# jzhoubu/vsearch

Hardware: AMD Instinct MI355X
Metric: queries/sec over 21M-doc sparse index, k=100; recall@100 vs reference (higher is better)
Workload: dtype f32

## Files before the change

### vsearch_amd/csrc/bp_quad.h

```cpp
#pragma once
#include "bp_walk.h"
#include "bp_quad_loop.h"
#include "bp_quad_asm.h"

#ifndef VS_QUAD_EPI
#define VS_QUAD_EPI 2
#endif

namespace vs {

constexpr int kQuadRows = 2048;
constexpr int kQuadQT = 8;
constexpr int kQuadPer = kBpEntCap / kScanThreads;
constexpr size_t kQuadAccBytes = (size_t)(kQuadRows / 16) * kQuadGroupDw * 4;
static_assert(kBpEntCap % kScanThreads == 0, "a thread owns a fixed number of entries");
static_assert(kQuadAccBytes >= kBpSortBytes, "the accumulator area holds the 8192-slot entry sort");
__host__ __device__ constexpr size_t quad_fixed_lds() { return kQuadAccBytes + (size_t)kBpCap * 8 + (size_t)kQuadQT * 16 + 64 * 4; }
__host__ __device__ constexpr size_t quad_cut_lds() { return quad_fixed_lds() + (size_t)(kBpEntCap + 64 + 64 * kQuadOverRead) * 8; }
__host__ __device__ constexpr size_t quad_lds_bytes() { return quad_cut_lds() + (size_t)kCutHistWords * 4; }
static_assert(quad_lds_bytes() <= (size_t)160 * 1024, "the quad walk's LDS");
static_assert(kBpCap == 2 * kScanThreads, "wg_cut_topk: two keys of the candidate buffer a thread");
static_assert(kQuadQT == 8 && (kQuadAccBytes + (size_t)kBpCap * 8) % 16 == 0, "the epilogue reads thresholds and counters 16 bytes at a time");
constexpr int kQuadListCap = 64 - 4 * kQuadOverRead, kQuadListBytes = (kQuadListCap + 4 * kQuadOverRead) * 8;
static_assert(kQuadListCap >= 16, "room for links in a wave's list");
static_assert(2 * kQuadListBytes * kScanWaves <= kBpCap * 8, "the link lists fit the sort buffer");
constexpr int kQuadLinked = kQuadCells - 2;
constexpr double kQuadMaxRatio = 3.0;
constexpr int kQuadPfLines = 384;
constexpr int kQuadPaceDefault = 0;
template <int CELLS, int LINKED>
__host__ __device__ constexpr uint32_t chunk_overflow(uint32_t n) { return n > (uint32_t)CELLS ? (n - (uint32_t)CELLS + (uint32_t)LINKED - 1u) / (uint32_t)LINKED : 0u; }
__host__ __device__ constexpr uint32_t quad_overflow_chunks(uint32_t n) { return chunk_overflow<kQuadCells, kQuadLinked>(n); }

template <int CELLS, int LINKED>
__global__ __launch_bounds__(kScanThreads) void quad_count_kernel(const uint32_t* pk_ptr, const uint4* cols, int64_t n_rows, int32_t n_cols, int32_t rows,
                                                                  uint32_t* dir, uint32_t* block_recs, unsigned long long* df_rec, unsigned long long* df_nnz,
                                                                  int32_t* overflow) {
    extern __shared__ __attribute__((aligned(16))) char smem[];
    uint32_t* cnt = reinterpret_cast<uint32_t*>(smem);
    __shared__ int scratch[32];
    const int tid = threadIdx.x;
    const int64_t n_blocks = (n_rows + rows - 1) / rows;
    const int seg = (n_cols + kScanThreads - 1) / kScanThreads;
    for (int64_t b = blockIdx.x; b < n_blocks; b += gridDim.x) {
        const int64_t r0 = b * rows, r1 = min(n_rows, r0 + rows);
        const uint32_t P0 = pk_ptr[r0], P1 = pk_ptr[r1];
        __syncthreads();
        for (int i = tid; i <= n_cols; i += kScanThreads) cnt[i] = 0;
        __syncthreads();
        for (uint32_t p = P0 + tid; p < P1; p += kScanThreads) {
            const uint4 cw = cols[p];
            const uint32_t cwv[4] = {cw.x, cw.y, cw.z, cw.w};
#pragma unroll
            for (int i = 0; i < 4; ++i) {
                atomicAdd(&cnt[cwv[i] & 0xFFFFu], 1u);
                atomicAdd(&cnt[cwv[i] >> 16], 1u);
            }
        }
        __syncthreads();
        const int i0 = min(n_cols, tid * seg), i1 = min(n_cols, i0 + seg);
        int mine = 0;
        for (int i = i0; i < i1; ++i) mine += (int)chunk_overflow<CELLS, LINKED>(cnt[i]);
        int tot = 0;
        int off = block_excl_scan(mine, scratch, tid, &tot);
        uint32_t* d = dir + (size_t)b * (n_cols + 1);
        for (int i = i0; i < i1; ++i) {
            const uint32_t c = cnt[i], r = chunk_overflow<CELLS, LINKED>(c);
            d[i] = bp_dir_pack((uint32_t)off, r);
            if (r > kBpDirRecMask || (uint32_t)off > kBpDirUnitMax) overflow[0] = 1;
            off += (int)r;
            atomicAdd(&df_rec[i], (unsigned long long)(1u + r));
            if (c) atomicAdd(&df_nnz[i], (unsigned long long)c);
        }
        if (tid == 0) { d[n_cols] = bp_dir_pack((uint32_t)tot, 0u); block_recs[b] = (uint32_t)n_cols + (uint32_t)tot; }
    }
}

template <int VS>
__global__ __launch_bounds__(kScanThreads) void quad_fill_kernel(const uint32_t* pk_ptr, const uint4* cols, const void* vals, int64_t n_rows, int32_t n_cols,
                                                                 int32_t rows, const uint32_t* dir, const unsigned long long* base, uint32_t* rec) {
    extern __shared__ __attribute__((aligned(16))) char smem[];
    uint32_t* cur = reinterpret_cast<uint32_t*>(smem);
    const int tid = threadIdx.x, lane = tid & 63, w = tid >> 6;
    const int64_t n_blocks = (n_rows + rows - 1) / rows;
    for (int64_t b = blockIdx.x; b < n_blocks; b += gridDim.x) {
        const int64_t r0 = b * rows, r1 = min(n_rows, r0 + rows);
        const uint32_t* d = dir + (size_t)b * (n_cols + 1);
        __syncthreads();
        for (int i = tid; i <= n_cols; i += kScanThreads) cur[i] = 0u;
        __syncthreads();
        uint32_t* brec = rec + (size_t)base[b] * kQuadCells;
        for (int64_t r = r0 + w; r < r1; r += kScanWaves) {
            const uint32_t p0 = pk_ptr[r], p1 = pk_ptr[r + 1];
            const uint32_t ai = quad_acc_index((uint32_t)(r - r0));
            for (uint32_t p = p0 + lane; p < p1; p += 64) {
                const uint4 cw = cols[p];
                const uint32_t cwv[4] = {cw.x, cw.y, cw.z, cw.w};
                uint32_t hb[8];
                if constexpr (VS == VM_F32) {
                    const float4* vp = reinterpret_cast<const float4*>(vals);
                    const float4 v0 = vp[2 * (size_t)p], v1 = vp[2 * (size_t)p + 1];
                    const float v[8] = {v0.x, v0.y, v0.z, v0.w, v1.x, v1.y, v1.z, v1.w};
#pragma unroll
                    for (int i = 0; i < 8; ++i) hb[i] = (uint32_t)__half_as_ushort(__float2half_rn(v[i]));
                } else {
                    const uint4 hv = reinterpret_cast<const uint4*>(vals)[p];
                    const uint32_t h4[4] = {hv.x, hv.y, hv.z, hv.w};
#pragma unroll
                    for (int i = 0; i < 8; ++i) hb[i] = (i & 1) ? (h4[i >> 1] >> 16) : (h4[i >> 1] & 0xFFFFu);
                }
#pragma unroll
                for (int i = 0; i < 8; ++i) {
                    const uint32_t c = (i & 1) ? (cwv[i >> 1] >> 16) : (cwv[i >> 1] & 0xFFFFu);
                    if (c < (uint32_t)n_cols) {
                        const uint32_t pos = atomicAdd(&cur[c], 1u);
                        const uint32_t w = d[c], m = w & kBpDirRecMask;
                        const uint32_t k = m ? min(pos / (uint32_t)kQuadLinked, m) : 0u;
                        const size_t chunk = k == 0 ? (size_t)c : (size_t)n_cols + (w >> 12) + (k - 1);
                        const uint32_t hv = (hb[i] & 0x7FFFu) ? hb[i] : 0u;
                        brec[chunk * kQuadCells + (pos - k * (uint32_t)kQuadLinked)] = ai | (hv << 16);
                    }
                }
            }
        }
        __syncthreads();
        for (int c = tid; c < n_cols; c += kScanThreads) {
            const uint32_t w = d[c], m = w & kBpDirRecMask;
            for (uint32_t k = 0; k < m; ++k) {
                const size_t chunk = k == 0 ? (size_t)c : (size_t)n_cols + (w >> 12) + (k - 1);
                const uint32_t link = (uint32_t)n_cols + (w >> 12) + k;
                brec[chunk * kQuadCells + 62] = (link >> 14) & 0x3FFFu;
                brec[chunk * kQuadCells + 63] = 0x80000000u | (link & 0x3FFFu);
            }
        }
    }
}

template <int UNUSED>
__global__ __launch_bounds__(256) void quad_arrange_kernel(uint32_t* rec, unsigned long long n_chunks) {
    extern __shared__ __attribute__((aligned(16))) char smem[];
    constexpr int LD = kQuadCells + 1;
    uint32_t* in = reinterpret_cast<uint32_t*>(smem);
    uint32_t* out = in + 256 * LD;
    const int tid = threadIdx.x;
    for (unsigned long long c0 = (unsigned long long)blockIdx.x * 256; c0 < n_chunks; c0 += (unsigned long long)gridDim.x * 256) {
        const int nc = (int)min((unsigned long long)256, n_chunks - c0);
        const uint4* src = reinterpret_cast<const uint4*>(rec + c0 * kQuadCells);
        __syncthreads();
        for (int i = tid; i < nc * 16; i += 256) {
            const uint4 v = src[i];
            uint32_t* q = in + (i >> 4) * LD + (i & 15) * 4;
            q[0] = v.x; q[1] = v.y; q[2] = v.z; q[3] = v.w;
        }
        __syncthreads();
        if (tid < nc) {
            const uint32_t* mi = in + tid * LD;
            uint32_t* mo = out + tid * LD;
            uint32_t mask[4] = {0u, 0u, 0u, 0u}, fill[4] = {0u, 0u, 0u, 0u}, room[4] = {16u, 16u, 16u, 16u};
            const bool linked = (mi[63] >> 31) != 0u;
            if (linked) {
                mo[62] = mi[62]; mo[63] = mi[63];
                mask[2] |= 1u << (mi[62] & 31u); mask[3] |= 1u << (mi[63] & 31u);
                room[2] = 15u; room[3] = 15u;
            }
            for (int i = 0; i < (linked ? kQuadLinked : kQuadCells); ++i) {
                const uint32_t p = mi[i];
                if ((p & 0x7FFF0000u) == 0u) continue;
                const uint32_t bit = 1u << (p & 31u);
                int pick = -1, any = -1;
                uint32_t best = 17u, best_any = 17u;
#pragma unroll
                for (int j = 0; j < 4; ++j) {
                    if (fill[j] < room[j] && fill[j] < best_any) { best_any = fill[j]; any = j; }
                    if (fill[j] < room[j] && !(mask[j] & bit) && fill[j] < best) { best = fill[j]; pick = j; }
                }
                if (pick < 0) pick = any;
#pragma unroll
                for (int j = 0; j < 4; ++j)
                    if (j == pick) { mo[fill[j] * 4 + j] = p; mask[j] |= bit; ++fill[j]; }
            }
#pragma unroll
            for (int j = 0; j < 4; ++j)
                while (fill[j] < room[j]) {
                    const uint32_t freeb = ~mask[j];
                    const uint32_t bk = freeb ? (uint32_t)(__ffs((int)freeb) - 1) : 0u;
                    mo[fill[j] * 4 + j] = quad_acc_index(bk);
                    mask[j] |= 1u << bk;
                    ++fill[j];
                }
        }
        __syncthreads();
        uint4* dst = reinterpret_cast<uint4*>(rec + c0 * kQuadCells);
        for (int i = tid; i < nc * 16; i += 256) {
            const uint32_t* q = out + (i >> 4) * LD + (i & 15) * 4;
            dst[i] = make_uint4(q[0], q[1], q[2], q[3]);
        }
    }
}

typedef unsigned short quad_us2 __attribute__((ext_vector_type(2)));

static_assert(kQuadRows <= 2 * kScanThreads && kQuadQT * 2 <= 32, "a thread's filter bits: two document rounds x the slots in one word");
constexpr int kQuadFiltWords = kQuadRows / 32 + 1;
constexpr size_t kQuadFiltStageBytes = (size_t)kQuadFiltWords * kQuadQT * 4;
static_assert(kQuadFiltWords * kQuadQT <= kScanThreads && quad_lds_bytes() + kQuadFiltStageBytes <= (size_t)160 * 1024, "the per-query filter stage");
template <int TM, int FL = 0>
__global__ __launch_bounds__(kScanThreads) void bp_quad_topk(KArg<BpArgs, FL> a) {
    constexpr int QT = kQuadQT;
    extern __shared__ __attribute__((aligned(16))) char smem[];
    int32_t* acc = reinterpret_cast<int32_t*>(smem);
    uint64_t* sortbuf = reinterpret_cast<uint64_t*>(smem + kQuadAccBytes);
    unsigned long long* tau = reinterpret_cast<unsigned long long*>(sortbuf + kBpCap);
    unsigned long long* upper_sh = tau + QT;
    int* scratch = reinterpret_cast<int*>(upper_sh + QT);
    unsigned int* ccnt = reinterpret_cast<unsigned int*>(scratch + 48);
    unsigned int* chi = ccnt + QT;
    uint2* desc = reinterpret_cast<uint2*>(scratch + 64);
    const uint32_t desc_lds = (uint32_t)quad_fixed_lds();
    uint32_t* cut_hist = reinterpret_cast<uint32_t*>(smem + quad_cut_lds());

    const int tid = threadIdx.x, lane = tid & 63, wv = tid >> 6;
    const int K = a.k;
    uint64_t* my_gcand = a.gcand + (size_t)blockIdx.x * QT * kBpCap;
    const int64_t n_blocks = (a.n_rows + a.rows - 1) / a.rows;
    const int64_t items = (int64_t)(a.n_tiles_dev ? a.n_tiles_dev[0] : a.n_tiles) * a.nchunk;
    const unsigned long long k_rt0 = TM ? __builtin_amdgcn_s_memrealtime() : 0ull;
    auto lds_barrier = [&]() { asm volatile("s_waitcnt lgkmcnt(0)\n\ts_barrier" ::: "memory"); };
    const uint32_t list_a = (uint32_t)kQuadAccBytes + (uint32_t)wv * 2u * kQuadListBytes, list_b = list_a + kQuadListBytes;
    const uint32_t g8 = (uint32_t)(lane >> 4) * 8u, s16 = (uint32_t)(lane & 15) * 16u;

    uint32_t pf_r = 0u, pf_R = 0u;
    if (a.pf_xcds > 0 && items <= (int64_t)gridDim.x && (int64_t)blockIdx.x < items) {
        const uint32_t X = (uint32_t)a.pf_xcds, R = ((uint32_t)items - blockIdx.x % X + X - 1u) / X;
        if (R >= 2u) { pf_r = blockIdx.x / X; pf_R = R; }
    }
    [[maybe_unused]] uint32_t n_coop = 0u;
    for (int64_t item = blockIdx.x; item < items; item += gridDim.x) {
        const int tile = (int)(item / a.nchunk), c = (int)(item % a.nchunk);
        const int q0 = a.tiles[tile].x, nq = a.tiles[tile].y;
        [[maybe_unused]] long long tm = TM ? (long long)__builtin_readcyclecounter() : 0;
        [[maybe_unused]] uint32_t tacc[6] = {0u, 0u, 0u, 0u, 0u, 0u};
        auto lap = [&](int phase) {
            if constexpr (TM != 0) {
                const long long now = (long long)__builtin_readcyclecounter();
                tacc[phase] += (uint32_t)(now - tm);
                tm = now;
            }
        };
        const int64_t b0 = (int64_t)c * a.blocks_per_chunk, b1 = min(n_blocks, b0 + a.blocks_per_chunk);
        __syncthreads();
        const int64_t e0 = a.qptr[q0], e1 = a.qptr[q0 + nq];
        const int n_ent = (int)(e1 - e0);
        const int n_static = (n_ent + 63) & ~63;
        {
            uint64_t* skey = reinterpret_cast<uint64_t*>(acc);
            for (int i = tid; i < 8192; i += kScanThreads) {
                uint64_t key = 0;
                if (i < n_ent) {
                    const int64_t e = e0 + i;
                    int qs = 0;
                    while (e >= a.qptr[q0 + qs + 1]) ++qs;
                    const float w = a.qvals[e] * a.qscale[q0 + qs];
                    key = ((uint64_t)1 << 63) | ((uint64_t)(uint32_t)a.qcols[e] << 40) | ((uint64_t)qs << 32) | (uint64_t)__float_as_uint(w);
                }
                skey[i] = key;
            }
            wg_sort_desc<kScanThreads>(skey, 8192, tid);
            for (int i = tid; i < n_static + 64 * kQuadOverRead; i += kScanThreads) {
                uint2 dsc = make_uint2(0u, 0u);
                if (i < n_ent) {
                    const uint64_t key = skey[i];
                    const uint32_t col = (uint32_t)(key >> 40) & 0xFFFFu, qs = (uint32_t)(key >> 32) & 0xFFu;
                    dsc = make_uint2((col << 8) | (qs * 16u), (uint32_t)key);
                }
                desc[i] = dsc;
            }
            __syncthreads();
        }
        for (int i = tid; i < (int)(kQuadAccBytes / 4); i += kScanThreads) acc[i] = 0;
        if (tid < QT) { tau[tid] = 0ull; ccnt[tid] = 0u; chi[tid] = 0u; }
        if (tid < QT) upper_sh[tid] = (a.upper && tid < nq) ? a.upper[q0 + tid] : ~0ull;
        __syncthreads();
        const uint32_t trips = (uint32_t)(n_static / 64);
        bool pace_off = false;
        unsigned long long base_cur = b0 < b1 ? a.base[b0] : 0ull;
        for (int64_t b = b0; b < b1 || b == b0; ++b) {
            const bool have = b < b1;
            const int rows_b = have ? (int)min((int64_t)a.rows, a.n_rows - b * a.rows) : 0;
            [[maybe_unused]] uint32_t fw0 = 0u, fw1 = 0u;
            if constexpr (FL != 0) {
                if (a.filt.ld == 0) {
                    const uint64_t bit = (uint64_t)(a.filt.bit0 + b * a.rows + tid);
                    if (tid < rows_b) fw0 = a.filt.words[bit >> 5];
                    if (tid + kScanThreads < rows_b) fw1 = a.filt.words[(bit + kScanThreads) >> 5];
                } else if (have) {
                    const int64_t w0 = (a.filt.bit0 + b * a.rows) >> 5, w1 = (a.filt.bit0 + b * a.rows + rows_b - 1) >> 5;
                    const int q = tid & (QT - 1), w = tid / QT;
                    if (w < kQuadFiltWords && q < nq && w0 + w <= w1) fw0 = a.filt.words[(size_t)(q0 + q) * (size_t)a.filt.ld + (size_t)(w0 + w)];
                }
            }
            if (have && trips > 0) {
                const char* brec = a.rec + (size_t)base_cur * kQuadChunkBytes;
                auto chain = [&](uint32_t n, uint32_t cur, uint32_t nxt) {
                    for (int depth = 0; n > 0 && depth < kQuadRows / kQuadLinked + 2; ++depth) {
                        const uint32_t n_pad = (n + 3u) & ~3u;
                        if ((uint32_t)lane < n_pad - n + 4u * kQuadOverRead)
                            reinterpret_cast<uint2*>(smem + cur)[n + (uint32_t)lane] = make_uint2(0u, 0u);
                        asm volatile("s_waitcnt lgkmcnt(0)" ::: "memory");
                        n = quad_list_asm(cur + g8, n_pad / 4u, brec, s16, nxt, (uint32_t)kQuadListCap);
                        const uint32_t t = cur; cur = nxt; nxt = t;
                    }
                };
                const uint32_t n_link = quad_walk_asm(desc_lds + (uint32_t)wv * 32u + g8, trips, brec, s16, list_a, (uint32_t)kQuadListCap);
                if (n_link <= (uint32_t)kQuadListCap) {
                    chain(n_link, list_a, list_b);
                } else {
                    constexpr uint32_t kSeg = kQuadListCap / 4;
                    for (uint32_t t0 = 0; t0 < trips; t0 += kSeg) {
                        const uint32_t n = quad_collect_asm(desc_lds + (uint32_t)wv * 32u + g8 + t0 * 512u, min(kSeg, trips - t0), brec, s16, list_a, (uint32_t)kQuadListCap);
                        chain(n, list_a, list_b);
                    }
                }
            }
            lap(1);
            if (a.pace && items <= (int64_t)gridDim.x && tid == 0 && have && !pace_off) {
                uint32_t* pc = a.pace + (size_t)c * a.blocks_per_chunk;
                const int64_t rel = b - b0;
                if (!((a.knob & 64) && blockIdx.x == 0))
                    __hip_atomic_fetch_add(pc + rel, 1u, __ATOMIC_RELAXED, __HIP_MEMORY_SCOPE_AGENT);
                if (rel >= a.pace_window) {
                    const uint32_t need = (uint32_t)(items / a.nchunk);
                    if (!pace_wait(pc + rel - a.pace_window, need)) pace_off = true;
                }
            }
            if (b + 1 < b1) base_cur = a.base[b + 1];
            if (a.gtau && tid < nq) { const unsigned long long g = a.gtau[q0 + tid]; if (g > tau[tid]) tau[tid] = g; }
            [[maybe_unused]] uint32_t fbits = 0u;
            [[maybe_unused]] uint32_t* fstage = reinterpret_cast<uint32_t*>(smem + quad_lds_bytes());
            if constexpr (FL != 0) {
                if (a.filt.ld == 0) {
#pragma unroll
                    for (int r = 0; r < 2; ++r) {
                        const uint64_t bit = (uint64_t)(a.filt.bit0 + b * a.rows + r * kScanThreads + tid);
                        if (r * kScanThreads + tid < rows_b && (((r ? fw1 : fw0) >> (bit & 31u)) & 1u)) fbits |= 0xFFu << (r * QT);
                    }
                } else if (tid < kQuadFiltWords * QT) {
                    fstage[tid] = fw0;
                }
                __builtin_amdgcn_s_waitcnt(0x0F70);
            }
            lds_barrier();
            if constexpr (FL != 0) {
                if (a.filt.ld != 0) {
                    const int64_t w0 = (a.filt.bit0 + b * a.rows) >> 5;
#pragma unroll
                    for (int r = 0; r < 2; ++r) {
                        const int d = r * kScanThreads + tid;
                        if (d < rows_b) {
                            const uint64_t bit = (uint64_t)(a.filt.bit0 + b * a.rows + d);
                            const uint4* p = reinterpret_cast<const uint4*>(fstage + ((int64_t)(bit >> 5) - w0) * QT);
                            const uint4 lo = p[0], hi = p[1];
                            const uint32_t w[QT] = {lo.x, lo.y, lo.z, lo.w, hi.x, hi.y, hi.z, hi.w};
#pragma unroll
                            for (int q = 0; q < QT; ++q) fbits |= ((w[q] >> (bit & 31u)) & 1u) << (r * QT + q);
                        }
                    }
                }
            }
            uint32_t pf = 0;
            if ((a.knob & 512) == 0 && b + 1 < b1 && trips > 0) {
                if (pf_R != 0u) {
                    const uint32_t L = pf_r + pf_R * (uint32_t)tid;
                    if (tid < a.pf_lines && L < 2u * (uint32_t)a.n_cols) {
                        const char* pl = a.rec + (size_t)base_cur * kQuadChunkBytes + (size_t)L * 128u;
                        asm volatile("global_load_dword %0, %1, off" : "=v"(pf) : "v"(pl) : "memory");
                    }
                    if constexpr (TM != 0) n_coop += 1u;
                } else if ((uint32_t)(lane >> 3) < trips) {
                    const uint32_t dx = *reinterpret_cast<const uint32_t*>(smem + desc_lds + (uint32_t)(lane >> 3) * 512u + (uint32_t)wv * 32u + (uint32_t)((lane >> 1) & 3) * 8u);
                    const char* pl = a.rec + (size_t)base_cur * kQuadChunkBytes + (dx & 0xFFFFFF00u) + (uint32_t)(lane & 1) * 128u;
                    asm volatile("global_load_dword %0, %1, off" : "=v"(pf) : "v"(pl) : "memory");
                }
            }
            lap(2);
            int32_t thr[QT];
            bool thr_stale = true;
            for (int d0 = 0; d0 < rows_b || d0 == 0; d0 += kScanThreads) {
                const int d = d0 + tid;
                const bool more = d0 + kScanThreads < rows_b;
                const uint32_t inc = more ? 1u : 0x10000u;
                if (d0 == 0 || thr_stale) {
                    const uint4* t4 = reinterpret_cast<const uint4*>(tau);
#pragma unroll
                    for (int i = 0; i < QT / 2; ++i) {
                        const uint4 t = t4[i];
                        thr[2 * i] = 2 * i < nq ? (int32_t)(t.y ^ 0x80000000u) : 0x7FFFFFFF;
                        thr[2 * i + 1] = 2 * i + 1 < nq ? (int32_t)(t.w ^ 0x80000000u) : 0x7FFFFFFF;
                    }
                    thr_stale = false;
                }
                if (d < rows_b) {
                    const int64_t row = b * a.rows + d;
                    int32_t sums[QT];
#if VS_QUAD_EPI == 0
                    int32_t* pa = acc + quad_acc_index((uint32_t)d);
#pragma unroll
                    for (int q = 0; q < QT; ++q) sums[q] = pa[q * 16];
#pragma unroll
                    for (int q = 0; q < QT; ++q) pa[q * 16] = 0;
#elif VS_QUAD_EPI == 1
                    {
                        const uint32_t pa = quad_acc_index((uint32_t)d) * 4u, zero = 0u;
                        asm volatile("ds_wrxchg_rtn_b32 %0, %8, %9\n\tds_wrxchg_rtn_b32 %1, %8, %9 offset:64\n\tds_wrxchg_rtn_b32 %2, %8, %9 offset:128\n\t"
                                     "ds_wrxchg_rtn_b32 %3, %8, %9 offset:192\n\tds_wrxchg_rtn_b32 %4, %8, %9 offset:256\n\tds_wrxchg_rtn_b32 %5, %8, %9 offset:320\n\t"
                                     "ds_wrxchg_rtn_b32 %6, %8, %9 offset:384\n\tds_wrxchg_rtn_b32 %7, %8, %9 offset:448\n\ts_waitcnt lgkmcnt(0)"
                                     : "=&v"(sums[0]), "=&v"(sums[1]), "=&v"(sums[2]), "=&v"(sums[3]), "=&v"(sums[4]), "=&v"(sums[5]), "=&v"(sums[6]), "=&v"(sums[7])
                                     : "v"(pa), "v"(zero) : "memory");
                    }
#else
                    {
                        const uint32_t pa = quad_acc_index((uint32_t)d) * 4u, zero = 0u;
                        unsigned long long s01, s23, s45, s67;
                        asm volatile("ds_wrxchg2_rtn_b32 %0, %4, %5, %5 offset0:0 offset1:16\n\tds_wrxchg2_rtn_b32 %1, %4, %5, %5 offset0:32 offset1:48\n\t"
                                     "ds_wrxchg2_rtn_b32 %2, %4, %5, %5 offset0:64 offset1:80\n\tds_wrxchg2_rtn_b32 %3, %4, %5, %5 offset0:96 offset1:112\n\ts_waitcnt lgkmcnt(0)"
                                     : "=&v"(s01), "=&v"(s23), "=&v"(s45), "=&v"(s67) : "v"(pa), "v"(zero) : "memory");
                        sums[0] = (int32_t)(uint32_t)s01; sums[1] = (int32_t)(uint32_t)(s01 >> 32); sums[2] = (int32_t)(uint32_t)s23; sums[3] = (int32_t)(uint32_t)(s23 >> 32);
                        sums[4] = (int32_t)(uint32_t)s45; sums[5] = (int32_t)(uint32_t)(s45 >> 32); sums[6] = (int32_t)(uint32_t)s67; sums[7] = (int32_t)(uint32_t)(s67 >> 32);
                    }
#endif
#pragma unroll
                    for (int q = 0; q < QT; ++q) {
                        if (sums[q] >= thr[q] && (FL == 0 || ((fbits >> ((d0 >= kScanThreads ? QT : 0) + q)) & 1u) != 0u)) {
                            const uint32_t hi = (uint32_t)sums[q] ^ 0x80000000u;
                            const uint64_t key = ((uint64_t)hi << 32) | (uint32_t)(~(uint32_t)row);
                            if (key > tau[q] && key < upper_sh[q]) {
                                const uint32_t old = atomicAdd(&ccnt[q], inc);
                                my_gcand[(size_t)q * kBpCap + (old & 0xFFFFu) + (old >> 16)] = key;
                            }
                        }
                    }
                }
                static_assert(kQuadRows <= 2 * kScanThreads, "the cut counter has two fields, first rounds | last round: a block is at most two epilogue rounds");
                lds_barrier();
                if ((a.knob & 128) && __builtin_amdgcn_readfirstlane(wv) == 5)
                    for (int i = 0; i < (a.knob >> 12); ++i) __builtin_amdgcn_s_sleep(8);
                const bool last = b + 1 >= b1 && !more;
                uint32_t cmax;
                {
                    const uint4* c4 = reinterpret_cast<const uint4*>(ccnt);
                    const uint4 c0 = c4[0], c1 = c4[1];
                    const uint32_t w[QT] = {c0.x, c0.y, c0.z, c0.w, c1.x, c1.y, c1.z, c1.w};
                    uint32_t t[QT];
                    if (more) {
                        const uint4 h0 = c4[2], h1 = c4[3];
                        const uint32_t h[QT] = {h0.x, h0.y, h0.z, h0.w, h1.x, h1.y, h1.z, h1.w};
#pragma unroll
                        for (int q = 0; q < QT; ++q) t[q] = __builtin_amdgcn_udot2(__builtin_bit_cast(quad_us2, w[q]), quad_us2{1, 0}, h[q], false);
                    } else {
#pragma unroll
                        for (int q = 0; q < QT; ++q) t[q] = __builtin_amdgcn_udot2(__builtin_bit_cast(quad_us2, w[q]), quad_us2{1, 1}, 0u, false);
                        if (tid < QT) chi[tid] = ccnt[tid] >> 16;
                    }
                    cmax = max(max(max(t[0], t[1]), max(t[2], t[3])), max(max(t[4], t[5]), max(t[6], t[7])));
                }
                const bool any = last || cmax > (uint32_t)(kBpCap - kScanThreads);
                [[maybe_unused]] long long t_cut = 0;
                if constexpr (TM != 0) t_cut = (long long)__builtin_readcyclecounter();
                if (any) __syncthreads();
                thr_stale = any;
                if (any)
                for (int qs = 0; qs < nq; ++qs) {
                    const uint32_t cw = ccnt[qs], cnt = (cw & 0xFFFFu) + (more ? chi[qs] : (cw >> 16));
                    if (last || cnt > (uint32_t)(kBpCap - kScanThreads)) {
                        for (int i = tid; i < kBpCap; i += kScanThreads) sortbuf[i] = (uint32_t)i < cnt ? my_gcand[(size_t)qs * kBpCap + i] : 0ull;
                        if (last) {
                            uint64_t* out = a.cand + ((size_t)(q0 + qs) * a.nchunk + c) * (size_t)K;
                            if (K <= 256) {
                                wg_final_topk256<kScanThreads>(sortbuf, cnt, K, my_gcand + (size_t)qs * kBpCap, out, cut_hist, tid);
                            } else {
                                wg_sort_desc<kScanThreads>(sortbuf, kBpCap, tid);
                                for (int i = tid; i < K; i += kScanThreads) out[i] = sortbuf[i];
                            }
                        } else if (cnt > (uint32_t)K) {
                            const unsigned long long kth_sel = wg_cut_topk<kScanThreads>(sortbuf, K, my_gcand + (size_t)qs * kBpCap, cut_hist, tid);
                            if (tid == 0) {
                                const unsigned long long kth = kth_sel;
                                if (kth > tau[qs]) tau[qs] = kth;
                                if (a.gtau && kth != 0ull) atomicMax(a.gtau + q0 + qs, kth);
                                ccnt[qs] = (uint32_t)K;
                                chi[qs] = 0u;
                            }
                        }
                        __syncthreads();
                    }
                }
                if constexpr (TM != 0) { if (any) tacc[3] += (uint32_t)((long long)__builtin_readcyclecounter() - t_cut); }
            }
            asm volatile("s_waitcnt vmcnt(0)" : "+v"(pf) : : "memory");
            lap(4);
            if constexpr (TM != 0) tacc[5] += 1u;
            if (b + 1 >= b1) break;
        }
        if constexpr (TM != 0) {
            if ((tid & 63) == 0) {
#pragma unroll
                for (int i = 0; i < 6; ++i) atomicAdd(a.timing + i, (unsigned long long)tacc[i]);
            }
        }
    }
    if (TM && threadIdx.x == 0) {
        if (n_coop) atomicAdd(a.timing + 10, (unsigned long long)n_coop);
        a.timing[16 + 4 * blockIdx.x] = __builtin_amdgcn_s_memrealtime() - k_rt0;
        a.timing[17 + 4 * blockIdx.x] = k_rt0;
        a.timing[18 + 4 * blockIdx.x] = (unsigned long long)__builtin_amdgcn_s_getreg((3 << 11) | 20);
        a.timing[19 + 4 * blockIdx.x] = (unsigned long long)__builtin_amdgcn_s_getreg((31 << 11) | 4);
    }
}

}
```

Measured before the change: 8113.

## Harvest both document rounds in one pass with a retry loop on candidate overflow

Adds a default-on one-pass epilogue. Each thread reads all eight thresholds and both of its documents' sixteen sums with batched ds_read2/ds_wrxchg2 instructions, then makes a wave-uniform ballot to skip candidate emission when nothing passes. Candidates that overflow the buffer stay pending and are retried after a cut, which replaces the two-round split counter and saves per-round barriers and threshold reloads. Inactive query slots get tau set to max so they never emit. The cost is more registers held live and a loop whose control flow is harder to follow.

```diff
diff --git a/vsearch_amd/csrc/bp_quad.h b/vsearch_amd/csrc/bp_quad.h
--- a/vsearch_amd/csrc/bp_quad.h
+++ b/vsearch_amd/csrc/bp_quad.h
@@ -5,6 +5,12 @@
 
 #ifndef VS_QUAD_EPI
 #define VS_QUAD_EPI 2
+#endif
+#ifndef VS_QUAD_HARVEST
+#define VS_QUAD_HARVEST 1
+#endif
+#if VS_QUAD_HARVEST == 1 && VS_QUAD_EPI != 2
+#error "the one-pass harvest reads a thread's sixteen sums with ds_wrxchg2_rtn_b32 (VS_QUAD_EPI=2)"
 #endif
 
 namespace vs {
@@ -214,7 +220,7 @@
     unsigned long long* upper_sh = tau + QT;
     int* scratch = reinterpret_cast<int*>(upper_sh + QT);
     unsigned int* ccnt = reinterpret_cast<unsigned int*>(scratch + 48);
-    unsigned int* chi = ccnt + QT;
+    [[maybe_unused]] unsigned int* chi = ccnt + QT;
     uint2* desc = reinterpret_cast<uint2*>(scratch + 64);
     const uint32_t desc_lds = (uint32_t)quad_fixed_lds();
     uint32_t* cut_hist = reinterpret_cast<uint32_t*>(smem + quad_cut_lds());
@@ -228,6 +234,9 @@
     auto lds_barrier = [&]() { asm volatile("s_waitcnt lgkmcnt(0)\n\ts_barrier" ::: "memory"); };
     const uint32_t list_a = (uint32_t)kQuadAccBytes + (uint32_t)wv * 2u * kQuadListBytes, list_b = list_a + kQuadListBytes;
     const uint32_t g8 = (uint32_t)(lane >> 4) * 8u, s16 = (uint32_t)(lane & 15) * 16u;
+    const uint32_t pa_doc = quad_acc_index((uint32_t)tid) * 4u;
+    constexpr uint32_t kSecondDoc = quad_acc_index((uint32_t)kScanThreads) * 4u;
+    static_assert(kScanThreads % 16 == 0, "document tid + 1024 is in the same place of its group of 16");
 
     uint32_t pf_r = 0u, pf_R = 0u;
     if (a.pf_xcds > 0 && items <= (int64_t)gridDim.x && (int64_t)blockIdx.x < items) {
@@ -278,7 +287,7 @@
             __syncthreads();
         }
         for (int i = tid; i < (int)(kQuadAccBytes / 4); i += kScanThreads) acc[i] = 0;
-        if (tid < QT) { tau[tid] = 0ull; ccnt[tid] = 0u; chi[tid] = 0u; }
+        if (tid < QT) { tau[tid] = tid < nq ? 0ull : ~0ull; ccnt[tid] = 0u; chi[tid] = 0u; }
         if (tid < QT) upper_sh[tid] = (a.upper && tid < nq) ? a.upper[q0 + tid] : ~0ull;
         __syncthreads();
         const uint32_t trips = (uint32_t)(n_static / 64);
@@ -383,6 +392,111 @@
                 }
             }
             lap(2);
+#if VS_QUAD_HARVEST == 1
+            {
+                int32_t thr[QT], sums[2][QT];
+                {
+                    const uint32_t pa1 = pa_doc + kSecondDoc, zero = 0u, tau_lds = (uint32_t)(kQuadAccBytes + (size_t)kBpCap * 8);
+                    unsigned long long t0, t1, t2, t3, s0, s1, s2, s3, s4, s5, s6, s7;
+                    asm volatile("ds_read2_b32 %0, %12 offset0:1 offset1:3\n\tds_read2_b32 %1, %12 offset0:5 offset1:7\n\t"
+                                 "ds_read2_b32 %2, %12 offset0:9 offset1:11\n\tds_read2_b32 %3, %12 offset0:13 offset1:15\n\t"
+                                 "ds_wrxchg2_rtn_b32 %4, %13, %15, %15 offset0:0 offset1:16\n\tds_wrxchg2_rtn_b32 %5, %13, %15, %15 offset0:32 offset1:48\n\t"
+                                 "ds_wrxchg2_rtn_b32 %6, %13, %15, %15 offset0:64 offset1:80\n\tds_wrxchg2_rtn_b32 %7, %13, %15, %15 offset0:96 offset1:112\n\t"
+                                 "ds_wrxchg2_rtn_b32 %8, %14, %15, %15 offset0:0 offset1:16\n\tds_wrxchg2_rtn_b32 %9, %14, %15, %15 offset0:32 offset1:48\n\t"
+                                 "ds_wrxchg2_rtn_b32 %10, %14, %15, %15 offset0:64 offset1:80\n\tds_wrxchg2_rtn_b32 %11, %14, %15, %15 offset0:96 offset1:112\n\ts_waitcnt lgkmcnt(0)"
+                                 : "=&v"(t0), "=&v"(t1), "=&v"(t2), "=&v"(t3), "=&v"(s0), "=&v"(s1), "=&v"(s2), "=&v"(s3), "=&v"(s4), "=&v"(s5), "=&v"(s6), "=&v"(s7)
+                                 : "v"(tau_lds), "v"(pa_doc), "v"(pa1), "v"(zero) : "memory");
+                    const unsigned long long tv[QT / 2] = {t0, t1, t2, t3}, sv[2][QT / 2] = {{s0, s1, s2, s3}, {s4, s5, s6, s7}};
+#pragma unroll
+                    for (int i = 0; i < QT / 2; ++i) {
+                        thr[2 * i] = (int32_t)((uint32_t)tv[i] ^ 0x80000000u);
+                        thr[2 * i + 1] = (int32_t)((uint32_t)(tv[i] >> 32) ^ 0x80000000u);
+#pragma unroll
+                        for (int r = 0; r < 2; ++r) { sums[r][2 * i] = (int32_t)(uint32_t)sv[r][i]; sums[r][2 * i + 1] = (int32_t)(uint32_t)(sv[r][i] >> 32); }
+                    }
+                }
+                bool hit = false;
+#pragma unroll
+                for (int r = 0; r < 2; ++r)
+#pragma unroll
+                    for (int q = 0; q < QT; ++q) hit = hit | (sums[r][q] >= thr[q]);
+                uint32_t pend = 0u;
+                if (__builtin_amdgcn_ballot_w64(hit) != 0ull) {
+                    uint32_t allow;
+                    if constexpr (FL != 0) allow = fbits;
+                    else allow = (tid < rows_b ? 0xFFu : 0u) | (tid + kScanThreads < rows_b ? 0xFF00u : 0u);
+#pragma unroll
+                    for (int i = 2 * QT - 1; i >= 0; --i) pend = (pend << 1) | (uint32_t)(sums[i / QT][i % QT] >= thr[i % QT]);
+                    pend &= allow;
+                }
+                const bool last = b + 1 >= b1;
+                for (;;) {
+                    if (__builtin_amdgcn_ballot_w64(pend != 0u) != 0ull) {
+                        uint32_t row_lo = (uint32_t)tid;
+                        asm volatile("" : "+v"(row_lo));
+                        row_lo = ~((uint32_t)(b * a.rows) + row_lo);
+#pragma unroll
+                        for (int r = 0; r < 2; ++r)
+#pragma unroll
+                            for (int q = 0; q < QT; ++q) {
+                                const uint32_t bit = 1u << (r * QT + q);
+                                if (pend & bit) {
+                                    uint32_t hi = (uint32_t)sums[r][q];
+                                    asm volatile("" : "+v"(hi));
+                                    const uint64_t key = ((uint64_t)(hi ^ 0x80000000u) << 32) | (uint32_t)(row_lo - (uint32_t)(r * kScanThreads));
+                                    bool keep = false;
+                                    if (key > tau[q] && key < upper_sh[q]) {
+                                        const uint32_t old = atomicAdd(&ccnt[q], 1u);
+                                        if (old < (uint32_t)kBpCap) my_gcand[(size_t)q * kBpCap + old] = key;
+                                        else keep = true;
+                                    }
+                                    if (!keep) pend &= ~bit;
+                                }
+                            }
+                    }
+                    lds_barrier();
+                    if ((a.knob & 128) && __builtin_amdgcn_readfirstlane(wv) == 5)
+                        for (int i = 0; i < (a.knob >> 12); ++i) __builtin_amdgcn_s_sleep(8);
+                    uint32_t cmax;
+                    {
+                        const uint4* c4 = reinterpret_cast<const uint4*>(ccnt);
+                        const uint4 c0 = c4[0], c1 = c4[1];
+                        cmax = max(max(max(c0.x, c0.y), max(c0.z, c0.w)), max(max(c1.x, c1.y), max(c1.z, c1.w)));
+                    }
+                    const bool over = cmax > (uint32_t)kBpCap;
+                    if (!(last || cmax > (uint32_t)(kBpCap - kScanThreads))) break;
+                    [[maybe_unused]] long long t_cut = 0;
+                    if constexpr (TM != 0) t_cut = (long long)__builtin_readcyclecounter();
+                    __syncthreads();
+                    for (int qs = 0; qs < nq; ++qs) {
+                        const uint32_t cw = ccnt[qs], cnt = min(cw, (uint32_t)kBpCap);
+                        if (last || cw > (uint32_t)(kBpCap - kScanThreads)) {
+                            for (int i = tid; i < kBpCap; i += kScanThreads) sortbuf[i] = (uint32_t)i < cnt ? my_gcand[(size_t)qs * kBpCap + i] : 0ull;
+                            if (last && !over) {
+                                uint64_t* out = a.cand + ((size_t)(q0 + qs) * a.nchunk + c) * (size_t)K;
+                                if (K <= 256) {
+                                    wg_final_topk256<kScanThreads>(sortbuf, cnt, K, my_gcand + (size_t)qs * kBpCap, out, cut_hist, tid);
+                                } else {
+                                    wg_sort_desc<kScanThreads>(sortbuf, kBpCap, tid);
+                                    for (int i = tid; i < K; i += kScanThreads) out[i] = sortbuf[i];
+                                }
+                            } else if (cnt > (uint32_t)K) {
+                                const unsigned long long kth_sel = wg_cut_topk<kScanThreads>(sortbuf, K, my_gcand + (size_t)qs * kBpCap, cut_hist, tid);
+                                if (tid == 0) {
+                                    const unsigned long long kth = kth_sel;
+                                    if (kth > tau[qs]) tau[qs] = kth;
+                                    if (a.gtau && kth != 0ull) atomicMax(a.gtau + q0 + qs, kth);
+                                    ccnt[qs] = (uint32_t)K;
+                                }
+                            }
+                            __syncthreads();
+                        }
+                    }
+                    if constexpr (TM != 0) tacc[3] += (uint32_t)((long long)__builtin_readcyclecounter() - t_cut);
+                    if (!over) break;
+                }
+            }
+#else
             int32_t thr[QT];
             bool thr_stale = true;
             for (int d0 = 0; d0 < rows_b || d0 == 0; d0 += kScanThreads) {
@@ -403,14 +517,14 @@
                     const int64_t row = b * a.rows + d;
                     int32_t sums[QT];
 #if VS_QUAD_EPI == 0
-                    int32_t* pa = acc + quad_acc_index((uint32_t)d);
+                    int32_t* pa = acc + (pa_doc + (d0 ? kSecondDoc : 0u)) / 4u;
 #pragma unroll
                     for (int q = 0; q < QT; ++q) sums[q] = pa[q * 16];
 #pragma unroll
                     for (int q = 0; q < QT; ++q) pa[q * 16] = 0;
 #elif VS_QUAD_EPI == 1
                     {
-                        const uint32_t pa = quad_acc_index((uint32_t)d) * 4u, zero = 0u;
+                        const uint32_t pa = pa_doc + (d0 ? kSecondDoc : 0u), zero = 0u;
                         asm volatile("ds_wrxchg_rtn_b32 %0, %8, %9\n\tds_wrxchg_rtn_b32 %1, %8, %9 offset:64\n\tds_wrxchg_rtn_b32 %2, %8, %9 offset:128\n\t"
                                      "ds_wrxchg_rtn_b32 %3, %8, %9 offset:192\n\tds_wrxchg_rtn_b32 %4, %8, %9 offset:256\n\tds_wrxchg_rtn_b32 %5, %8, %9 offset:320\n\t"
                                      "ds_wrxchg_rtn_b32 %6, %8, %9 offset:384\n\tds_wrxchg_rtn_b32 %7, %8, %9 offset:448\n\ts_waitcnt lgkmcnt(0)"
@@ -419,7 +533,7 @@
                     }
 #else
                     {
-                        const uint32_t pa = quad_acc_index((uint32_t)d) * 4u, zero = 0u;
+                        const uint32_t pa = pa_doc + (d0 ? kSecondDoc : 0u), zero = 0u;
                         unsigned long long s01, s23, s45, s67;
                         asm volatile("ds_wrxchg2_rtn_b32 %0, %4, %5, %5 offset0:0 offset1:16\n\tds_wrxchg2_rtn_b32 %1, %4, %5, %5 offset0:32 offset1:48\n\t"
                                      "ds_wrxchg2_rtn_b32 %2, %4, %5, %5 offset0:64 offset1:80\n\tds_wrxchg2_rtn_b32 %3, %4, %5, %5 offset0:96 offset1:112\n\ts_waitcnt lgkmcnt(0)"
@@ -428,16 +542,23 @@
                         sums[4] = (int32_t)(uint32_t)s45; sums[5] = (int32_t)(uint32_t)(s45 >> 32); sums[6] = (int32_t)(uint32_t)s67; sums[7] = (int32_t)(uint32_t)(s67 >> 32);
                     }
 #endif
+                    bool hit = false;
+#pragma unroll
+                    for (int q = 0; q < QT; ++q) hit = hit | (sums[q] >= thr[q]);
+                    if (__builtin_amdgcn_ballot_w64(hit) != 0ull) {
+                    [[maybe_unused]] const uint32_t fb = d0 ? fbits >> QT : fbits;
+                    const uint32_t row_lo = ~(uint32_t)row;
 #pragma unroll
                     for (int q = 0; q < QT; ++q) {
-                        if (sums[q] >= thr[q] && (FL == 0 || ((fbits >> ((d0 >= kScanThreads ? QT : 0) + q)) & 1u) != 0u)) {
+                        if (sums[q] >= thr[q] && (FL == 0 || ((fb >> q) & 1u) != 0u)) {
                             const uint32_t hi = (uint32_t)sums[q] ^ 0x80000000u;
-                            const uint64_t key = ((uint64_t)hi << 32) | (uint32_t)(~(uint32_t)row);
+                            const uint64_t key = ((uint64_t)hi << 32) | row_lo;
                             if (key > tau[q] && key < upper_sh[q]) {
                                 const uint32_t old = atomicAdd(&ccnt[q], inc);
                                 my_gcand[(size_t)q * kBpCap + (old & 0xFFFFu) + (old >> 16)] = key;
                             }
                         }
+                    }
                     }
                 }
                 static_assert(kQuadRows <= 2 * kScanThreads, "the cut counter has two fields, first rounds | last round: a block is at most two epilogue rounds");
@@ -496,6 +617,7 @@
                 }
                 if constexpr (TM != 0) { if (any) tacc[3] += (uint32_t)((long long)__builtin_readcyclecounter() - t_cut); }
             }
+#endif
             asm volatile("s_waitcnt vmcnt(0)" : "+v"(pf) : : "memory");
             lap(4);
             if constexpr (TM != 0) tacc[5] += 1u;
```

After: 8283, median of 6. +2.1%, better.
